# Syclus123/xDeepFM-pytorch

Hardware: AMD Instinct MI355X
Metric: examples/sec (xDeepFM train step, Criteo-shape synthetic, bs=4096 per GPU) (higher is better)
Workload: dtype f32

## Files before the change

### xdeepfm-pytorch_amd/csrc/adam.hip

```cpp
#include "xdfm_internal.h"
#include "finish_batch.h"
#include "adam_math.h"
#include "cin_x3_pack.h"
#include "table_step.h"

#define ADAM_THREADS 256
#define ADAM_BX 512
#define ADAM_BLOCK_ELEMS 8192
#define ADAM_FLUSH_BX 4096



#define ADAM_CHUNK 64
struct AdamDev {
    float* param; float* grad; float* exp_avg; float* exp_avg_sq; const float* step; unsigned char* grad_marks; unsigned char* last;
    long numel; float l2; int flags;
};
static inline AdamDev adam_dev(const xdfm_adam_tensor& t) {
    return AdamDev{t.param, t.grad, t.exp_avg, t.exp_avg_sq, t.step, t.grad_marks, t.last, t.numel, t.l2, t.flags};
}
struct AdamBatch { AdamDev t[ADAM_CHUNK]; int first[ADAM_CHUNK + 1]; };
static_assert(sizeof(AdamBatch) + 128 <= 8192, "the Adam kernels' argument block");

template <bool NT>
// ... 184 lines not shown
__global__ void adam_tick_kernel(int* __restrict__ clock, float* __restrict__ consts, int cap, double lr_arg,
                                 const double* __restrict__ lr_dev, double beta1, double beta2) {
    if (threadIdx.x != 0 || blockIdx.x != 0) return;
    const double lr = lr_dev ? *lr_dev : lr_arg;
    int t = clock[0] + 1;
    if (t >= cap) t = cap - 1;
    clock[0] = t;
    const double step = (double)(clock[1] + t);
    const float ss = (float)(lr / (1.0 - pow(beta1, step)));
    const float bc = (float)sqrt(1.0 - pow(beta2, step));
    const bool ok = bc >= 0.00390625f && bc <= 1.f && ss >= 9.313225746154785e-10f && ss <= 1024.f;
    float* k = consts + ADAM_CONSTS_PER_STEP * t;
    k[0] = ss;
    k[1] = bc;
    k[2] = bc * 4294967296.f;
    k[3] = ok ? adam_exact_rcp(bc) * 2.3283064365386963e-10f : 0.f;
}

__global__ void adam_clock_reset_kernel(int* __restrict__ clock) {
    if (threadIdx.x == 0 && blockIdx.x == 0) { clock[1] += clock[0]; clock[0] = 0; }
}

__device__ __forceinline__ long long adam_backlog_fix(float v) { return (long long)((double)v * ADAM_FIX); }
__device__ __forceinline__ void adam_backlog_add_fix(long long f, unsigned long long* __restrict__ backlog) {
    for (int o = 32; o > 0; o >>= 1) f += __shfl_xor(f, o);
    __shared__ long long part[ADAM_THREADS / 64];
    if ((threadIdx.x & 63) == 0) part[threadIdx.x >> 6] = f;
    __syncthreads();
    if (threadIdx.x == 0) {
        long long tot = 0;
        for (int k = 0; k < ADAM_THREADS / 64; ++k) tot += part[k];
        if (tot) atomicAdd(backlog, (unsigned long long)tot);
    }
}
__device__ __forceinline__ void adam_backlog_add(float v, unsigned long long* __restrict__ backlog) {
    adam_backlog_add_fix(adam_backlog_fix(v), backlog);
}

struct AdamRowsDev {
    float* const* p; float* const* m; float* const* v; unsigned char* const* last; const float* l2;
    float* const* g; unsigned char* const* marks;
};
__device__ __forceinline__ AdamRowsDev adam_rows_pick(bool is_lin, const AdamRowsDev& emb, const AdamRowsDev& lin) {
    AdamRowsDev R;
    R.p = is_lin ? lin.p : emb.p; R.m = is_lin ? lin.m : emb.m; R.v = is_lin ? lin.v : emb.v;
    R.last = is_lin ? lin.last : emb.last; R.l2 = is_lin ? lin.l2 : emb.l2;
    R.g = is_lin ? lin.g : emb.g; R.marks = is_lin ? lin.marks : emb.marks;
    return R;
}

struct AdamClaim { int f; long cc; int old; bool is_lin; };
__device__ __forceinline__ AdamClaim adam_claim_chunk(long idx, const float* __restrict__ X, long ldx, const int* __restrict__ cols,
                                                      const int* __restrict__ vocab, int m, int D, int QE, int QT,
                                                      const AdamRowsDev& emb, const AdamRowsDev& lin, int t, bool need_table) {
    AdamClaim k;
    const int q = (int)(idx % QT);
    const long r = idx / QT;
    k.f = (int)(r % m);
    const long b = r / m;
    const int V = vocab[k.f];
    long id = (long)X[b * ldx + cols[k.f]];
    if (id < 0 || id >= V) id = id < 0 ? 0 : V - 1;
    k.is_lin = q >= QE;
    const AdamRowsDev R = adam_rows_pick(k.is_lin, emb, lin);
    const long w = k.is_lin ? 1 : D;
    const long c0 = id * w / 4, c1 = (id * w + w - 1) / 4;
    k.cc = c0 + (k.is_lin ? 0 : q);
    const long n4 = (long)V * w / 4;
    k.old = -1;
    if (k.cc <= c1 && k.cc < n4 && (!need_table || R.p[k.f] != nullptr))
        k.old = tbl_claim(R.last[k.f], k.cc, t);
    return k;
}

__global__ __launch_bounds__(ADAM_THREADS) void adam_catchup_rows_kernel(
    const float* __restrict__ X, long ldx, int B, const int* __restrict__ cols, const int* __restrict__ vocab, int m, int D,
    AdamRowsDev emb, AdamRowsDev lin, int has_lin, const int* __restrict__ clock, const float* __restrict__ consts,
    double beta1, double beta2, double eps, unsigned long long* __restrict__ backlog, int own_blocks, const X3PackJobs riders) {
    if ((int)blockIdx.x >= own_blocks) { x3_absmax_rider(riders, (long)((int)blockIdx.x - own_blocks)); return; }
    const int t = clock[0];
    const int QE = (D + 3) / 4 + ((D & 3) ? 1 : 0);
    const int QT = QE + (has_lin ? 1 : 0);
    const long idx = (long)blockIdx.x * ADAM_THREADS + threadIdx.x;
    const AdamCoef c = {(float)(1.0 - beta1), (float)beta2, (float)(1.0 - beta2), 0.f, (float)eps};
    const bool eps_ok = c.eps >= ADAM_EPS_MIN && c.eps <= 1.f;
    float zf;
    asm volatile("v_mov_b32 %0, 0" : "=v"(zf));
    AdamClaim k;
    k.old = -1; k.f = 0; k.cc = 0; k.is_lin = false;
    if (t > 0 && idx < (long)B * m * QT) k = adam_claim_chunk(idx, X, ldx, cols, vocab, m, D, QE, QT, emb, lin, t, false);
    const bool act = k.old >= 0;
    const AdamRowsDev R = adam_rows_pick(k.is_lin, emb, lin);
    float4 pa = make_float4(0.f, 0.f, 0.f, 0.f), ma = pa, va = pa;
    float4 *p4 = nullptr, *m4 = nullptr, *v4 = nullptr;
    float l2c = 0.f;
    if (act) {
        p4 = reinterpret_cast<float4*>(R.p[k.f]) + k.cc;
        m4 = reinterpret_cast<float4*>(R.m[k.f]) + k.cc;
        v4 = reinterpret_cast<float4*>(R.v[k.f]) + k.cc;
        pa = *p4; ma = *m4; va = *v4;
        l2c = R.l2[k.f];
    }
    adam_f2 sq2 = {0.f, 0.f};
    adam_replay_span(pa, ma, va, act, k.old, t, consts, 2.f * l2c, zf, c, sq2, eps_ok);
    if (act) { *p4 = pa; *m4 = ma; *v4 = va; }
    adam_backlog_add(l2c * (sq2.x + sq2.y), backlog);
}

__device__ __forceinline__ void adam_apply_rows_body(
    const float* __restrict__ X, long ldx, int B, const int* __restrict__ cols, const int* __restrict__ vocab, int m, int D,
    const AdamRowsDev emb, const AdamRowsDev lin, int has_lin, const int* __restrict__ clock, const float* __restrict__ consts,
    double beta1, double beta2, double eps, unsigned long long* __restrict__ cell, const long bid) {
    const int t = clock[0];
    const int QE = (D + 3) / 4 + ((D & 3) ? 1 : 0);
    const int QT = QE + (has_lin ? 1 : 0);
    const long idx = bid * ADAM_THREADS + threadIdx.x;
    const long nrow = (long)B * m * QT;
    const float ss = consts[ADAM_CONSTS_PER_STEP * t], bc = consts[ADAM_CONSTS_PER_STEP * t + 1];
    const AdamCoef c = {(float)(1.0 - beta1), (float)beta2, (float)(1.0 - beta2), 0.f, (float)eps};
    const bool eps_ok = c.eps >= ADAM_EPS_MIN && c.eps <= 1.f;
    float zf;
    asm volatile("v_mov_b32 %0, 0" : "=v"(zf));
    float sqv = 0.f;
    AdamClaim k;
    k.old = -1; k.f = 0; k.cc = 0; k.is_lin = false;
    if (idx < nrow) k = adam_claim_chunk(idx, X, ldx, cols, vocab, m, D, QE, QT, emb, lin, t, true);
    const bool act = k.old >= 0;
    {
        const AdamRowsDev R = adam_rows_pick(k.is_lin, emb, lin);
        float4 pa = make_float4(0.f, 0.f, 0.f, 0.f), ma = pa, va = pa, ga = pa;
        float4 *p4 = nullptr, *m4 = nullptr, *v4 = nullptr;
        float l2c = 0.f;
        if (act) {
            p4 = reinterpret_cast<float4*>(R.p[k.f]) + k.cc;
            m4 = reinterpret_cast<float4*>(R.m[k.f]) + k.cc;
            v4 = reinterpret_cast<float4*>(R.v[k.f]) + k.cc;
            float4* g4 = reinterpret_cast<float4*>(R.g[k.f]) + k.cc;
            pa = *p4; ma = *m4; va = *v4; ga = *g4;
            *g4 = make_float4(zf, zf, zf, zf);
            R.marks[k.f][k.cc] = 0;
            l2c = R.l2[k.f];
        }
        const float g2 = 2.f * l2c;
        adam_f2 sq2 = {0.f, 0.f};
        adam_replay_span(pa, ma, va, act, k.old, t - 1, consts, g2, zf, c, sq2, eps_ok);
        if (act) {
            float sq = sq2.x + sq2.y;
            adam_four(pa, ma, va, ga, g2, ss, bc, c, sq);
            *p4 = pa; *m4 = ma; *v4 = va;
            sqv = l2c * sq;
        }
    }
    if (idx >= nrow && idx < nrow + 8L * m) {
        const long u = idx - nrow;
        const int kk = (int)(u & 3);
        const int f = (int)((u >> 2) % m);
        const bool is_lin = (u >> 2) >= m;
        if (!is_lin || has_lin) {
            const AdamRowsDev R = adam_rows_pick(is_lin, emb, lin);
            const long numel = (long)vocab[f] * (is_lin ? 1 : D);
            const long e = numel / 4 * 4 + kk;
            if (e < numel && R.p[f] != nullptr) {
                float* p = R.p[f]; float* mm = R.m[f]; float* vv = R.v[f]; float* g = R.g[f];
                const float l2c = R.l2[f];
                float pa = p[e], ma = mm[e], va = vv[e];
                sqv = l2c * (pa * pa);
                adam_one(pa, fmaf(2.f * l2c, pa, g[e]), ma, va, ss, bc, c);
                p[e] = pa; mm[e] = ma; vv[e] = va;
                g[e] = 0.f;
                R.marks[f][e >> 2] = 0;
            }
        }
    }
    adam_backlog_add(sqv, cell);
}
__global__ __launch_bounds__(ADAM_THREADS) void adam_apply_rows_kernel(
    const float* __restrict__ X, long ldx, int B, const int* __restrict__ cols, const int* __restrict__ vocab, int m, int D,
    AdamRowsDev emb, AdamRowsDev lin, int has_lin, const int* __restrict__ clock, const float* __restrict__ consts,
    double beta1, double beta2, double eps, unsigned long long* __restrict__ cell) {
    adam_apply_rows_body(X, ldx, B, cols, vocab, m, D, emb, lin, has_lin, clock, consts, beta1, beta2, eps, cell, (long)blockIdx.x);
}

struct AdamRow { int f; long c0; int nq; bool is_lin; };
__device__ __forceinline__ AdamRow adam_row_of(long idx, bool live, const float* __restrict__ X, long ldx, const int* __restrict__ cols,
                                               const int* __restrict__ vocab, int m, int B, int D, int has_lin) {
    AdamRow r;
    r.f = 0; r.c0 = 0; r.nq = 0; r.is_lin = false;
    const long nE = (long)m * B;
    if (!live || idx >= (has_lin ? 2 * nE : nE)) return r;
    r.is_lin = idx >= nE;
    const long u = r.is_lin ? idx - nE : idx;
    r.f = (int)(u / B);
    const long b = u - (long)r.f * B;
    const int V = vocab[r.f];
    long id = (long)X[b * ldx + cols[r.f]];
    if (id < 0 || id >= V) id = id < 0 ? 0 : V - 1;
    const long w = r.is_lin ? 1 : D;
    r.c0 = id * w / 4;
    const long left = (long)V * w / 4 - r.c0;
    const long want = r.is_lin ? 1 : D / 4;
    r.nq = (int)(left < want ? (left > 0 ? left : 0) : want);
    return r;
}
__device__ __forceinline__ unsigned long long adam_row_claim(const AdamRow& r, unsigned char* last, int q0, int t) {
    const int gn = r.nq - q0 < 8 ? r.nq - q0 : 8;
    if (gn <= 0) return ~0ull;
    if (!r.is_lin) return tbl_claim_row(last, r.c0 + q0, gn, t);
    const int old = tbl_claim(last, r.c0, t);
    return old < 0 ? ~0ull : ((~0ull << 8) | (unsigned long long)old);
}

__global__ __launch_bounds__(ADAM_THREADS) void adam_catchup_by_row_kernel(
    const float* __restrict__ X, long ldx, int B, const int* __restrict__ cols, const int* __restrict__ vocab, int m, int D,
    AdamRowsDev emb, AdamRowsDev lin, int has_lin, const int* __restrict__ clock, const float* __restrict__ consts,
    double beta1, double beta2, double eps, unsigned long long* __restrict__ backlog, int own_blocks, const X3PackJobs riders) {
    if ((int)blockIdx.x >= own_blocks) { x3_absmax_rider(riders, (long)((int)blockIdx.x - own_blocks)); return; }
    const int t = clock[0];
    const int Q = D / 4;
    const long idx = (long)blockIdx.x * ADAM_THREADS + threadIdx.x;
    const AdamCoef c = {(float)(1.0 - beta1), (float)beta2, (float)(1.0 - beta2), 0.f, (float)eps};
    const bool eps_ok = c.eps >= ADAM_EPS_MIN && c.eps <= 1.f;
    float zf;
    asm volatile("v_mov_b32 %0, 0" : "=v"(zf));
    const AdamRow r = adam_row_of(idx, t > 0, X, ldx, cols, vocab, m, B, D, has_lin);
    const AdamRowsDev R = adam_rows_pick(r.is_lin, emb, lin);
    float4 *p4 = nullptr, *m4 = nullptr, *v4 = nullptr;
    unsigned char* last = nullptr;
    float l2c = 0.f;
    if (r.nq > 0) {
        p4 = reinterpret_cast<float4*>(R.p[r.f]) + r.c0;
        m4 = reinterpret_cast<float4*>(R.m[r.f]) + r.c0;
        v4 = reinterpret_cast<float4*>(R.v[r.f]) + r.c0;
        last = R.last[r.f];
        l2c = R.l2[r.f];
    }
    long long fix = 0;
    for (int q0 = 0; q0 < Q; q0 += 8) {
        const unsigned long long olds = adam_row_claim(r, last, q0, t);
        const int turns = Q - q0 < 8 ? Q - q0 : 8;
        for (int j = 0; j < turns; ++j) {
            const int old = (int)((olds >> (8 * j)) & 255ull);
            const bool act = old != 255;
            float4 pa = make_float4(0.f, 0.f, 0.f, 0.f), ma = pa, va = pa;
            if (act) { pa = p4[q0 + j]; ma = m4[q0 + j]; va = v4[q0 + j]; }
            adam_f2 sq2 = {0.f, 0.f};
            adam_replay_span(pa, ma, va, act, old, t, consts, 2.f * l2c, zf, c, sq2, eps_ok);
            if (act) {
                p4[q0 + j] = pa; m4[q0 + j] = ma; v4[q0 + j] = va;
                fix += adam_backlog_fix(l2c * (sq2.x + sq2.y));
            }
        }
    }
    adam_backlog_add_fix(fix, backlog);
}

__device__ __forceinline__ void adam_apply_by_row_body(
    const float* __restrict__ X, long ldx, int B, const int* __restrict__ cols, const int* __restrict__ vocab, int m, int D,
    const AdamRowsDev emb, const AdamRowsDev lin, int has_lin, const int* __restrict__ clock, const float* __restrict__ consts,
    double beta1, double beta2, double eps, unsigned long long* __restrict__ cell, const long bid) {
    const int t = clock[0];
    const int Q = D / 4;
    const long idx = bid * ADAM_THREADS + threadIdx.x;
    const long nrow = (long)B * m * (has_lin ? 2 : 1);
    const float ss = consts[ADAM_CONSTS_PER_STEP * t], bc = consts[ADAM_CONSTS_PER_STEP * t + 1];
    const AdamCoef c = {(float)(1.0 - beta1), (float)beta2, (float)(1.0 - beta2), 0.f, (float)eps};
    const bool eps_ok = c.eps >= ADAM_EPS_MIN && c.eps <= 1.f;
    float zf;
    asm volatile("v_mov_b32 %0, 0" : "=v"(zf));
    long long fix = 0;
    {
        AdamRow r = adam_row_of(idx, true, X, ldx, cols, vocab, m, B, D, has_lin);
        const AdamRowsDev R = adam_rows_pick(r.is_lin, emb, lin);
        float4 *p4 = nullptr, *m4 = nullptr, *v4 = nullptr, *g4 = nullptr;
        unsigned char *last = nullptr, *marks = nullptr;
        float l2c = 0.f;
        if (r.nq > 0 && R.p[r.f] == nullptr) r.nq = 0;
        if (r.nq > 0) {
            p4 = reinterpret_cast<float4*>(R.p[r.f]) + r.c0;
            m4 = reinterpret_cast<float4*>(R.m[r.f]) + r.c0;
            v4 = reinterpret_cast<float4*>(R.v[r.f]) + r.c0;
            g4 = reinterpret_cast<float4*>(R.g[r.f]) + r.c0;
            marks = R.marks[r.f] + r.c0;
            last = R.last[r.f];
            l2c = R.l2[r.f];
        }
        const float g2 = 2.f * l2c;
        for (int q0 = 0; q0 < Q; q0 += 8) {
            const unsigned long long olds = adam_row_claim(r, last, q0, t);
            const int turns = Q - q0 < 8 ? Q - q0 : 8;
            for (int j = 0; j < turns; ++j) {
                const int old = (int)((olds >> (8 * j)) & 255ull);
                const bool act = old != 255;
                float4 pa = make_float4(0.f, 0.f, 0.f, 0.f), ma = pa, va = pa, ga = pa;
                if (act) {
                    pa = p4[q0 + j]; ma = m4[q0 + j]; va = v4[q0 + j]; ga = g4[q0 + j];
                    g4[q0 + j] = make_float4(zf, zf, zf, zf);
                    marks[q0 + j] = 0;
                }
                adam_f2 sq2 = {0.f, 0.f};
                adam_replay_span(pa, ma, va, act, old, t - 1, consts, g2, zf, c, sq2, eps_ok);
                if (act) {
                    float sq = sq2.x + sq2.y;
                    adam_four(pa, ma, va, ga, g2, ss, bc, c, sq);
                    p4[q0 + j] = pa; m4[q0 + j] = ma; v4[q0 + j] = va;
                    fix += adam_backlog_fix(l2c * sq);
                }
            }
        }
    }
    if (idx >= nrow && idx < nrow + 8L * m) {
        const long u = idx - nrow;
        const int kk = (int)(u & 3);
        const int f = (int)((u >> 2) % m);
        const bool is_lin = (u >> 2) >= m;
        if (!is_lin || has_lin) {
            const AdamRowsDev R = adam_rows_pick(is_lin, emb, lin);
            const long numel = (long)vocab[f] * (is_lin ? 1 : D);
            const long e = numel / 4 * 4 + kk;
            if (e < numel && R.p[f] != nullptr) {
                float* p = R.p[f]; float* mm = R.m[f]; float* vv = R.v[f]; float* g = R.g[f];
                const float l2c = R.l2[f];
                float pa = p[e], ma = mm[e], va = vv[e];
                fix += adam_backlog_fix(l2c * (pa * pa));
                adam_one(pa, fmaf(2.f * l2c, pa, g[e]), ma, va, ss, bc, c);
                p[e] = pa; mm[e] = ma; vv[e] = va;
                g[e] = 0.f;
                R.marks[f][e >> 2] = 0;
            }
        }
    }
    adam_backlog_add_fix(fix, cell);
}
__global__ __launch_bounds__(ADAM_THREADS) void adam_apply_by_row_kernel(
    const float* __restrict__ X, long ldx, int B, const int* __restrict__ cols, const int* __restrict__ vocab, int m, int D,
    AdamRowsDev emb, AdamRowsDev lin, int has_lin, const int* __restrict__ clock, const float* __restrict__ consts,
    double beta1, double beta2, double eps, unsigned long long* __restrict__ cell) {
    adam_apply_by_row_body(X, ldx, B, cols, vocab, m, D, emb, lin, has_lin, clock, consts, beta1, beta2, eps, cell, (long)blockIdx.x);
}

struct AdamRowsArgs {
    const float* X; long ldx; int B; const int* cols; const int* vocab; int m; int D;
    AdamRowsDev emb, lin; int has_lin; unsigned long long* cell;
};
static_assert(sizeof(AdamBatch) + sizeof(AdamRowsArgs) + 128 <= 8192, "adam_step_rows_kernel's argument block");
template <bool BY_ROW>
__global__ __launch_bounds__(ADAM_THREADS, 3) void adam_step_rows_kernel(
    const AdamBatch batch, int cnt, int slot0, double lr_arg, const double* __restrict__ lr_dev, double beta1, double beta2, double eps,
    float* __restrict__ l2_part, const int* __restrict__ clock, const float* __restrict__ consts, const AdamRowsArgs r) {
    const int own = batch.first[cnt];
    if ((int)blockIdx.x < own) {
        adam_step_body<true>(batch, cnt, slot0, lr_arg, lr_dev, beta1, beta2, eps, l2_part, clock, consts, (int)blockIdx.x);
        return;
    }
    const long bid = (long)blockIdx.x - own;
    if constexpr (BY_ROW)
        adam_apply_by_row_body(r.X, r.ldx, r.B, r.cols, r.vocab, r.m, r.D, r.emb, r.lin, r.has_lin, clock, consts, beta1, beta2, eps, r.cell, bid);
    else
        adam_apply_rows_body(r.X, r.ldx, r.B, r.cols, r.vocab, r.m, r.D, r.emb, r.lin, r.has_lin, clock, consts, beta1, beta2, eps, r.cell, bid);
}

__global__ void adam_rows_finish_kernel(unsigned long long* __restrict__ cell, float* __restrict__ l2_value) {
    if (threadIdx.x == 0 && blockIdx.x == 0) adam_rows_finish_one(cell, l2_value);
}
int xdfm_adam_rows_finish(unsigned long long* cell, float* l2_value, hipStream_t st) {
    FinishJob j{};
    j.kind = FJ_ADAM_ROWS; j.blocks = 1;
    j.cell = cell; j.out = l2_value;
    bool taken = false;
    if (int rc = xdfm_finish_defer(j, st, &taken)) return rc;
    if (!taken) hipLaunchKernelGGL(adam_rows_finish_kernel, dim3(1), dim3(64), 0, st, cell, l2_value);
    return XDFM_OK;
}

__global__ __launch_bounds__(ADAM_THREADS) void adam_flush_kernel(const AdamBatch batch, int cnt, const int* __restrict__ clock,
                                                                  const float* __restrict__ consts, double beta1, double beta2,
                                                                  double eps, unsigned long long* __restrict__ backlog) {
    int ti = 0;
    for (int k = 1; k < cnt; ++k) ti += (int)blockIdx.x >= batch.first[k] ? 1 : 0;
    const int lb = (int)blockIdx.x - batch.first[ti];
    const int nb = batch.first[ti + 1] - batch.first[ti];
    const AdamDev& d = batch.t[ti];
    const int t = clock[0];
    float4* p4 = reinterpret_cast<float4*>(d.param);
    float4* m4 = reinterpret_cast<float4*>(d.exp_avg);
    float4* v4 = reinterpret_cast<float4*>(d.exp_avg_sq);
    unsigned char* __restrict__ last = d.last;
    const long n4 = d.numel / 4;
    const float l2c = d.l2;
    const float g2 = 2.f * l2c;
    float zf;
    asm volatile("v_mov_b32 %0, 0" : "=v"(zf));
    const AdamCoef c = {(float)(1.0 - beta1), (float)beta2, (float)(1.0 - beta2), 0.f, (float)eps};
    adam_f2 sq2 = {0.f, 0.f};
    const bool eps_ok = c.eps >= ADAM_EPS_MIN && c.eps <= 1.f;
    for (long base = (long)lb * ADAM_THREADS; base < n4; base += (long)nb * ADAM_THREADS) {
        const long i = base + threadIdx.x;
        const bool in = i < n4;
        const int old = in ? (int)last[i] : 0;
        const bool act = in && old < t;
        float4 pa = make_float4(0.f, 0.f, 0.f, 0.f), ma = pa, va = pa;
        if (act) { pa = tbl_ld<true>(p4 + i); ma = tbl_ld<true>(m4 + i); va = tbl_ld<true>(v4 + i); }
        adam_replay_span(pa, ma, va, act, old, t, consts, g2, zf, c, sq2, eps_ok);
        if (act) { tbl_st<true>(p4 + i, pa); tbl_st<true>(m4 + i, ma); tbl_st<true>(v4 + i, va); }
        if (in && old) last[i] = 0;
    }
    adam_backlog_add(l2c * (sq2.x + sq2.y), backlog);
}

__device__ __forceinline__ unsigned long long adam_mix(unsigned long long z) {
    z += 0x9e3779b97f4a7c15ull;
    z = (z ^ (z >> 30)) * 0xbf58476d1ce4e5b9ull;
    z = (z ^ (z >> 27)) * 0x94d049bb133111ebull;
    return z ^ (z >> 31);
}
__device__ __forceinline__ float adam_rand_float(unsigned long long h, int emin, int emax, bool sign) {
    const int e = emin + (int)((h >> 32) % (unsigned)(emax - emin));
    const unsigned bits = ((unsigned)(e + 127) << 23) | ((unsigned)h & 0x7fffffu) | ((sign && ((h >> 60) & 1)) ? 0x80000000u : 0u);
    return __uint_as_float(bits);
}
__device__ __forceinline__ AdamStepConst adam_const_for(double lr, double beta1, double beta2, double step) {
    AdamStepConst k;
    k.ss = (float)(lr / (1.0 - pow(beta1, step)));
    k.bc = (float)sqrt(1.0 - pow(beta2, step));
    k.c2 = k.bc * 4294967296.f;
    k.rc2 = adam_exact_rcp(k.bc) * 2.3283064365386963e-10f;
    return k;
}
__global__ __launch_bounds__(256) void adam_selftest_kernel(int mode, unsigned long long base, unsigned long long n,
                                                            unsigned long long seed, double lr, double beta1, double beta2, double eps,
                                                            unsigned long long* __restrict__ out) {
#pragma clang fp contract(off)
    const unsigned long long idx = base + (unsigned long long)blockIdx.x * 256 + threadIdx.x;
    unsigned long long bad = 0, done = 0, what = 0;
    if (idx < n) {
        if (mode == 0) {
            const float x = __uint_as_float((unsigned)idx);
            if (x > 0.f && x < ADAM_V_MAX) {
                const float x2 = x * 18446744073709551616.f;
                const float fast = adam_sqrt_scaled2(adam_f2{x2, x2}).x, ref = sqrtf(x) * 4294967296.f;
                done = 1; bad = __float_as_uint(fast) != __float_as_uint(ref); what = idx;
            }
        } else if (mode == 1) {
            const unsigned mant = (unsigned)(idx & 0xffffffull);
            const unsigned long long tt = (idx >> 24) + 1;
            const float bc = tt <= 256 ? (float)sqrt(1.0 - pow(beta2, (double)tt)) : adam_rand_float(adam_mix(seed + tt), -8, 0, false);
            const float S = __uint_as_float(0x3f800000u + mant);
            const float s2 = S * 4294967296.f;
            const float fast = adam_div_const2(adam_f2{s2, s2}, bc * 4294967296.f, adam_exact_rcp(bc) * 2.3283064365386963e-10f).y;
            const float ref = S / bc;
            done = 1; bad = __float_as_uint(fast) != __float_as_uint(ref); what = idx;
        } else if (mode == 2) {
            const unsigned long long h0 = adam_mix(seed + 2 * idx), h1 = adam_mix(seed + 2 * idx + 1);
            const float d = adam_rand_float(h0, -40, 40, false);
            float nn = adam_rand_float(h1, -80, 40, true);
            if ((h1 >> 40) % 1021 == 0) nn = 0.f;
            if ((h1 >> 40) % 1021 == 1) nn = __uint_as_float(((h0 >> 61) & 1) ? 0x17800000u : 0x537fffffu);
            const float fast = adam_div2(adam_f2{nn, nn}, adam_f2{d, d}).x, ref = nn / d;
            done = 1; bad = __float_as_uint(fast) != __float_as_uint(ref) && !(fast == 0.f && ref == 0.f);
            what = ((unsigned long long)__float_as_uint(nn) << 32) | __float_as_uint(d);
        } else {
            const AdamCoef c = {(float)(1.0 - beta1), (float)beta2, (float)(1.0 - beta2), 0.f, (float)eps};
            const bool eps_ok = c.eps >= ADAM_EPS_MIN && c.eps <= 1.f;
            float zf;
            asm volatile("v_mov_b32 %0, 0" : "=v"(zf));
            float pv[4], mv[4], vv[4];
            for (int e = 0; e < 4; ++e) {
                const unsigned long long h = adam_mix(seed + 16 * idx + e), h2 = adam_mix(h), h3 = adam_mix(h2);
                pv[e] = adam_rand_float(h, -30, 8, true);
                mv[e] = adam_rand_float(h2, -60, 4, true);
                vv[e] = adam_rand_float(h3, -100, 10, false);
                const unsigned sel = (unsigned)((h >> 48) % 97);
                if (sel == 0) pv[e] = 0.f;
                if (sel == 1) { mv[e] = 0.f; vv[e] = 0.f; }
                if (sel == 2) pv[e] = __uint_as_float(0x00000fffu);
                if (sel == 3) { pv[e] = 3e30f; vv[e] = 1e35f; }
                if (sel == 4) mv[e] = __uint_as_float(0x00400000u);
                if (sel == 5) vv[e] = __uint_as_float(0x00000001u);
            }
            const float g2 = (adam_mix(seed + idx) & 7) == 0 ? 0.f : 2e-5f;
            float4 pf = make_float4(pv[0], pv[1], pv[2], pv[3]), mf = make_float4(mv[0], mv[1], mv[2], mv[3]),
                   vf = make_float4(vv[0], vv[1], vv[2], vv[3]);
            for (int st = 1; st <= 6 && !bad; ++st) {
                const AdamStepConst k = adam_const_for(lr, beta1, beta2, (double)(st + (idx % 50) * 7));
                float4 pr = pf, mr = mf, vr = vf;
                adam_f2 sq2 = {0.f, 0.f};
                adam_replay4(pf, mf, vf, k, g2, zf, c, sq2, eps_ok);
                float* a[3] = {&pr.x, &mr.x, &vr.x};
                for (int e = 0; e < 4; ++e) adam_one(a[0][e], fmaf(g2, a[0][e], zf), a[1][e], a[2][e], k.ss, k.bc, c);
                const float* f[3] = {&pf.x, &mf.x, &vf.x};
                for (int q = 0; q < 3; ++q)
                    for (int e = 0; e < 4; ++e) {
                        const float x = f[q][e], y = a[q][e];
                        if (__float_as_uint(x) != __float_as_uint(y) && !(x != x && y != y) && !(x == 0.f && y == 0.f)) bad = 1;
                    }
                done += 1;
                what = idx * 8 + st;
            }
        }
    }
    if (done) atomicAdd(&out[0], done);
    if (bad) { atomicAdd(&out[1], 1ull); atomicMax(&out[2], what); }
}

static int adam_clock_ok(const char* what, const xdfm_adam_clock* clk) {
    XDFM_REQUIRE(clk && clk->clock && clk->consts && clk->cap > 2 && clk->cap <= 256, "%s: bad clock", what);
    return XDFM_OK;
}

static bool adam_by_row(int D) {
    const bool by_row = D % 4 == 0 && xdfm_opt(OPT_ADAM_ROWS) != 0;
    xdfm_opt_note(OPT_LAST_ADAM_ROWS, by_row ? 1 : 0);
    return by_row;
}

extern "C" {

size_t xdfm_adam_step_ws_elems(int T) { return T > 0 ? (size_t)T * ADAM_BX : 0; }

int xdfm_adam_step(const xdfm_adam_tensor* tensors, int T, double lr, double beta1, double beta2, double eps,
                   float* l2_ws, float* l2_value, void* stream) {
    return xdfm_adam_step_lr(tensors, T, lr, nullptr, beta1, beta2, eps, l2_ws, l2_value, stream);
}

static int adam_step_impl(const xdfm_adam_tensor* tensors, int T, const xdfm_adam_clock* clk, double lr, const double* lr_dev,
                          double beta1, double beta2, double eps, float* l2_ws, float* l2_value, void* stream,
                          const AdamRowsArgs* rows = nullptr, bool rows_by_row = false, int rows_blocks = 0);

int xdfm_adam_step_lr(const xdfm_adam_tensor* tensors, int T, double lr, const double* lr_dev, double beta1, double beta2,
                      double eps, float* l2_ws, float* l2_value, void* stream) {
    return adam_step_impl(tensors, T, nullptr, lr, lr_dev, beta1, beta2, eps, l2_ws, l2_value, stream);
}

int xdfm_adam_step_deferred(const xdfm_adam_tensor* tensors, int T, const xdfm_adam_clock* clk, double lr,
                            const double* lr_dev, double beta1, double beta2, double eps, float* l2_ws, float* l2_value,
                            void* stream) {
    XDFM_REQUIRE(!(clk && clk->clock && clk->consts && clk->cap > 256), "adam_step_deferred: bad clock (cap %d > 256)", clk->cap);
    if (int rc = adam_clock_ok("adam_step_deferred", clk)) return rc;
    return adam_step_impl(tensors, T, clk, lr, lr_dev, beta1, beta2, eps, l2_ws, l2_value, stream);
}

static int adam_step_impl(const xdfm_adam_tensor* tensors, int T, const xdfm_adam_clock* clk, double lr, const double* lr_dev,
                          double beta1, double beta2, double eps, float* l2_ws, float* l2_value, void* stream,
                          const AdamRowsArgs* rows, bool rows_by_row, int rows_blocks) {
    if (int rc = tbl_check_call("adam_step", tensors, T)) return rc;
// ... 164 lines not shown
```

### xdeepfm-pytorch_amd/csrc/adam_math.h

```cpp
#pragma once
#include <hip/hip_runtime.h>

typedef float adam_f2 __attribute__((ext_vector_type(2)));

struct AdamCoef { float w1, b2, w2, lr, eps; };

__device__ __forceinline__ void adam_one(float& p, float g, float& m, float& v, float step_size, float bc2_sqrt, const AdamCoef& c) {
#pragma clang fp contract(off)
    m = fmaf(c.w1, g - m, m);
    v = fmaf(c.w2 * g, g, c.b2 * v);
    const float denom = sqrtf(v) / bc2_sqrt + c.eps;
    p -= step_size * m / denom;
}

__device__ __forceinline__ void adam_four(float4& pa, float4& ma, float4& va, float4 ga, float g2, float step_size, float bc2_sqrt,
                                          const AdamCoef& c, float& sq) {
    sq += (pa.x * pa.x + pa.y * pa.y) + (pa.z * pa.z + pa.w * pa.w);
    ga.x = fmaf(g2, pa.x, ga.x); ga.y = fmaf(g2, pa.y, ga.y); ga.z = fmaf(g2, pa.z, ga.z); ga.w = fmaf(g2, pa.w, ga.w);
    adam_one(pa.x, ga.x, ma.x, va.x, step_size, bc2_sqrt, c); adam_one(pa.y, ga.y, ma.y, va.y, step_size, bc2_sqrt, c);
    adam_one(pa.z, ga.z, ma.z, va.z, step_size, bc2_sqrt, c); adam_one(pa.w, ga.w, ma.w, va.w, step_size, bc2_sqrt, c);
}

struct AdamStepConst { float ss, bc, c2, rc2; };
#define ADAM_CONSTS_PER_STEP 4

__device__ __forceinline__ adam_f2 adam_pkfma(adam_f2 a, adam_f2 b, adam_f2 c) { return __builtin_elementwise_fma(a, b, c); }

__device__ __forceinline__ adam_f2 adam_sqrt_scaled2(adam_f2 x2) {
#pragma clang fp contract(off)
    adam_f2 y;
    y.x = __builtin_amdgcn_rsqf(x2.x);
    y.y = __builtin_amdgcn_rsqf(x2.y);
    const adam_f2 half = {0.5f, 0.5f};
    const adam_f2 s0 = x2 * y, h0 = half * y;
    const adam_f2 r = adam_pkfma(-s0, h0, half);
    const adam_f2 s1 = adam_pkfma(s0, r, s0), h1 = adam_pkfma(h0, r, h0);
    const adam_f2 dd = adam_pkfma(-s1, s1, x2);
    return adam_pkfma(dd, h1, s1);
}

__device__ __forceinline__ adam_f2 adam_div_const2(adam_f2 s, float c2, float rc2) {
#pragma clang fp contract(off)
    const adam_f2 C = {c2, c2}, R = {rc2, rc2};
    const adam_f2 t0 = s * R;
    const adam_f2 r0 = adam_pkfma(-t0, C, s);
    const adam_f2 t1 = adam_pkfma(r0, R, t0);
    const adam_f2 r1 = adam_pkfma(-t1, C, s);
    return adam_pkfma(r1, R, t1);
}

__device__ __forceinline__ adam_f2 adam_div2(adam_f2 n, adam_f2 d) {
#pragma clang fp contract(off)
    adam_f2 y0;
    y0.x = __builtin_amdgcn_rcpf(d.x);
    y0.y = __builtin_amdgcn_rcpf(d.y);
    const adam_f2 one = {1.f, 1.f};
    const adam_f2 e = adam_pkfma(-d, y0, one);
    const adam_f2 y1 = adam_pkfma(e, y0, y0);
    const adam_f2 q0 = n * y1;
    const adam_f2 r0 = adam_pkfma(-d, q0, n);
    const adam_f2 q1 = adam_pkfma(r0, y1, q0);
    const adam_f2 r1 = adam_pkfma(-d, q1, n);
    return adam_pkfma(r1, y1, q1);
}

#define ADAM_V_MAX 4.611686018427388e18f
#define ADAM_M_MIN 8.881784197001252e-16f
#define ADAM_M_MAX 1073741824.0f
#define ADAM_EPS_MIN 9.094947017729282e-13f

__device__ __forceinline__ void adam_replay4(float4& p, float4& m, float4& v, const AdamStepConst& k, float g2, float zf,
                                             const AdamCoef& c, adam_f2& sq2, bool eps_ok) {
#pragma clang fp contract(off)
    adam_f2 pa = {p.x, p.y}, pb = {p.z, p.w};
    sq2 += adam_pkfma(pb, pb, pa * pa);
    const adam_f2 G2 = {g2, g2}, Z = {zf, zf}, W1 = {c.w1, c.w1}, W2 = {c.w2, c.w2}, B2 = {c.b2, c.b2};
    const adam_f2 ga = adam_pkfma(G2, pa, Z), gb = adam_pkfma(G2, pb, Z);
    adam_f2 ma = {m.x, m.y}, mb = {m.z, m.w}, va = {v.x, v.y}, vb = {v.z, v.w};
    const adam_f2 ma1 = adam_pkfma(W1, ga - ma, ma), mb1 = adam_pkfma(W1, gb - mb, mb);
    const adam_f2 va1 = adam_pkfma(W2 * ga, ga, B2 * va), vb1 = adam_pkfma(W2 * gb, gb, B2 * vb);
    const float vmin = fminf(fminf(va1.x, va1.y), fminf(vb1.x, vb1.y)), vmax = fmaxf(fmaxf(va1.x, va1.y), fmaxf(vb1.x, vb1.y));
    const float mmin = fminf(fminf(fabsf(ma1.x), fabsf(ma1.y)), fminf(fabsf(mb1.x), fabsf(mb1.y)));
    const float mmax = fmaxf(fmaxf(fabsf(ma1.x), fabsf(ma1.y)), fmaxf(fabsf(mb1.x), fabsf(mb1.y)));
    const bool fast = vmin > 0.f && vmax < ADAM_V_MAX && mmin >= ADAM_M_MIN && mmax < ADAM_M_MAX;
    if (eps_ok && k.rc2 != 0.f && __builtin_amdgcn_ballot_w64(!fast) == 0) {
        const adam_f2 big = {18446744073709551616.f, 18446744073709551616.f};
        const adam_f2 E = {c.eps, c.eps}, SS = {k.ss, k.ss};
        const adam_f2 sa = adam_sqrt_scaled2(va1 * big), sb = adam_sqrt_scaled2(vb1 * big);
        const adam_f2 da = adam_div_const2(sa, k.c2, k.rc2) + E, db = adam_div_const2(sb, k.c2, k.rc2) + E;
        const adam_f2 neg1 = {-1.f, -1.f};
        pa = adam_pkfma(adam_div2(SS * ma1, da), neg1, pa);
        pb = adam_pkfma(adam_div2(SS * mb1, db), neg1, pb);
        p = make_float4(pa.x, pa.y, pb.x, pb.y);
        m = make_float4(ma1.x, ma1.y, mb1.x, mb1.y);
        v = make_float4(va1.x, va1.y, vb1.x, vb1.y);
    } else {
        adam_one(p.x, ga.x, m.x, v.x, k.ss, k.bc, c); adam_one(p.y, ga.y, m.y, v.y, k.ss, k.bc, c);
        adam_one(p.z, gb.x, m.z, v.z, k.ss, k.bc, c); adam_one(p.w, gb.y, m.w, v.w, k.ss, k.bc, c);
    }
}

__device__ __forceinline__ AdamStepConst adam_step_const(const float* __restrict__ consts, int s) {
    const float4 t = *reinterpret_cast<const float4*>(consts + ADAM_CONSTS_PER_STEP * s);
    return AdamStepConst{t.x, t.y, t.z, t.w};
}

__device__ __forceinline__ void adam_replay_span(float4& p, float4& m, float4& v, bool active, int old, int t_end,
                                                 const float* __restrict__ consts, float g2, float zf, const AdamCoef& c,
                                                 adam_f2& sq2, bool eps_ok) {
    int mn = active ? old : 0x7fffffff;
    for (int o = 32; o > 0; o >>= 1) {
        const int other = __shfl_xor(mn, o);
        mn = other < mn ? other : mn;
    }
    const int first = __builtin_amdgcn_readfirstlane(mn);
    if (first >= t_end) return;
    for (int s = first + 1; s <= t_end; ++s) {
        const AdamStepConst k = adam_step_const(consts, s);
        if (active && s > old) adam_replay4(p, m, v, k, g2, zf, c, sq2, eps_ok);
    }
}

__host__ __device__ inline float adam_exact_rcp(float c) {
    float y = (float)(1.0 / (double)c);
    double best = fabs(1.0 - (double)c * (double)y);
    const float cand[2] = {nextafterf(y, 0.f), nextafterf(y, 3.0e38f)};
    float out = y;
    for (int k = 0; k < 2; ++k) {
        const double r = fabs(1.0 - (double)c * (double)cand[k]);
        if (r < best) { best = r; out = cand[k]; }
    }
    return out;
}
```

Before: 2.184 million.

## Restructure Adam replay math into interleaved packed pairs with uniform coefficients

Reworks the lazy-Adam replay inner step so the sqrt, constant-divide and divide refinements process two packed float pairs side by side, with sched barriers forcing the two chains to interleave. The fast-path range checks become integer bit comparisons combined through wave ballots, and the coefficients are forced into scalar registers with readfirstlane. The full-table flush kernel gains a uniform-loop variant that skips the per-step activity check when all active lanes share the same start step, and it addresses through a shared base plus a lane offset. These changes target ALU latency and VGPR pressure in the catch-up path. The cost is more code and a schedule pinned by barriers, which could stop the compiler from finding a better ordering.

```diff
diff --git a/xdeepfm-pytorch_amd/csrc/adam.hip b/xdeepfm-pytorch_amd/csrc/adam.hip
--- a/xdeepfm-pytorch_amd/csrc/adam.hip
+++ b/xdeepfm-pytorch_amd/csrc/adam.hip
@@ -290,7 +290,7 @@
     const int QE = (D + 3) / 4 + ((D & 3) ? 1 : 0);
     const int QT = QE + (has_lin ? 1 : 0);
     const long idx = (long)blockIdx.x * ADAM_THREADS + threadIdx.x;
-    const AdamCoef c = {(float)(1.0 - beta1), (float)beta2, (float)(1.0 - beta2), 0.f, (float)eps};
+    const AdamCoef c = adam_uniform(AdamCoef{(float)(1.0 - beta1), (float)beta2, (float)(1.0 - beta2), 0.f, (float)eps});
     const bool eps_ok = c.eps >= ADAM_EPS_MIN && c.eps <= 1.f;
     float zf;
     asm volatile("v_mov_b32 %0, 0" : "=v"(zf));
@@ -325,7 +325,7 @@
     const long idx = bid * ADAM_THREADS + threadIdx.x;
     const long nrow = (long)B * m * QT;
     const float ss = consts[ADAM_CONSTS_PER_STEP * t], bc = consts[ADAM_CONSTS_PER_STEP * t + 1];
-    const AdamCoef c = {(float)(1.0 - beta1), (float)beta2, (float)(1.0 - beta2), 0.f, (float)eps};
+    const AdamCoef c = adam_uniform(AdamCoef{(float)(1.0 - beta1), (float)beta2, (float)(1.0 - beta2), 0.f, (float)eps});
     const bool eps_ok = c.eps >= ADAM_EPS_MIN && c.eps <= 1.f;
     float zf;
     asm volatile("v_mov_b32 %0, 0" : "=v"(zf));
@@ -426,7 +426,7 @@
     const int t = clock[0];
     const int Q = D / 4;
     const long idx = (long)blockIdx.x * ADAM_THREADS + threadIdx.x;
-    const AdamCoef c = {(float)(1.0 - beta1), (float)beta2, (float)(1.0 - beta2), 0.f, (float)eps};
+    const AdamCoef c = adam_uniform(AdamCoef{(float)(1.0 - beta1), (float)beta2, (float)(1.0 - beta2), 0.f, (float)eps});
     const bool eps_ok = c.eps >= ADAM_EPS_MIN && c.eps <= 1.f;
     float zf;
     asm volatile("v_mov_b32 %0, 0" : "=v"(zf));
@@ -471,7 +471,7 @@
     const long idx = bid * ADAM_THREADS + threadIdx.x;
     const long nrow = (long)B * m * (has_lin ? 2 : 1);
     const float ss = consts[ADAM_CONSTS_PER_STEP * t], bc = consts[ADAM_CONSTS_PER_STEP * t + 1];
-    const AdamCoef c = {(float)(1.0 - beta1), (float)beta2, (float)(1.0 - beta2), 0.f, (float)eps};
+    const AdamCoef c = adam_uniform(AdamCoef{(float)(1.0 - beta1), (float)beta2, (float)(1.0 - beta2), 0.f, (float)eps});
     const bool eps_ok = c.eps >= ADAM_EPS_MIN && c.eps <= 1.f;
     float zf;
     asm volatile("v_mov_b32 %0, 0" : "=v"(zf));
@@ -595,21 +595,22 @@
     unsigned char* __restrict__ last = d.last;
     const long n4 = d.numel / 4;
     const float l2c = d.l2;
-    const float g2 = 2.f * l2c;
+    const float g2 = adam_uniform(2.f * l2c);
     float zf;
     asm volatile("v_mov_b32 %0, 0" : "=v"(zf));
-    const AdamCoef c = {(float)(1.0 - beta1), (float)beta2, (float)(1.0 - beta2), 0.f, (float)eps};
+    const AdamCoef c = adam_uniform(AdamCoef{(float)(1.0 - beta1), (float)beta2, (float)(1.0 - beta2), 0.f, (float)eps});
     adam_f2 sq2 = {0.f, 0.f};
     const bool eps_ok = c.eps >= ADAM_EPS_MIN && c.eps <= 1.f;
+    const unsigned tx16 = threadIdx.x * 16u;
     for (long base = (long)lb * ADAM_THREADS; base < n4; base += (long)nb * ADAM_THREADS) {
         const long i = base + threadIdx.x;
         const bool in = i < n4;
         const int old = in ? (int)last[i] : 0;
         const bool act = in && old < t;
         float4 pa = make_float4(0.f, 0.f, 0.f, 0.f), ma = pa, va = pa;
-        if (act) { pa = tbl_ld<true>(p4 + i); ma = tbl_ld<true>(m4 + i); va = tbl_ld<true>(v4 + i); }
-        adam_replay_span(pa, ma, va, act, old, t, consts, g2, zf, c, sq2, eps_ok);
-        if (act) { tbl_st<true>(p4 + i, pa); tbl_st<true>(m4 + i, ma); tbl_st<true>(v4 + i, va); }
+        if (act) { pa = tbl_ld<true>(at4(p4 + base, tx16)); ma = tbl_ld<true>(at4(m4 + base, tx16)); va = tbl_ld<true>(at4(v4 + base, tx16)); }
+        adam_replay_span<true>(pa, ma, va, act, old, t, consts, g2, zf, c, sq2, eps_ok);
+        if (act) { tbl_st<true>(at4(p4 + base, tx16), pa); tbl_st<true>(at4(m4 + base, tx16), ma); tbl_st<true>(at4(v4 + base, tx16), va); }
         if (in && old) last[i] = 0;
     }
     adam_backlog_add(l2c * (sq2.x + sq2.y), backlog);
@@ -667,7 +668,7 @@
             done = 1; bad = __float_as_uint(fast) != __float_as_uint(ref) && !(fast == 0.f && ref == 0.f);
             what = ((unsigned long long)__float_as_uint(nn) << 32) | __float_as_uint(d);
         } else {
-            const AdamCoef c = {(float)(1.0 - beta1), (float)beta2, (float)(1.0 - beta2), 0.f, (float)eps};
+            const AdamCoef c = adam_uniform(AdamCoef{(float)(1.0 - beta1), (float)beta2, (float)(1.0 - beta2), 0.f, (float)eps});
             const bool eps_ok = c.eps >= ADAM_EPS_MIN && c.eps <= 1.f;
             float zf;
             asm volatile("v_mov_b32 %0, 0" : "=v"(zf));
diff --git a/xdeepfm-pytorch_amd/csrc/adam_math.h b/xdeepfm-pytorch_amd/csrc/adam_math.h
--- a/xdeepfm-pytorch_amd/csrc/adam_math.h
+++ b/xdeepfm-pytorch_amd/csrc/adam_math.h
@@ -5,12 +5,24 @@
 
 struct AdamCoef { float w1, b2, w2, lr, eps; };
 
-__device__ __forceinline__ void adam_one(float& p, float g, float& m, float& v, float step_size, float bc2_sqrt, const AdamCoef& c) {
+__device__ __forceinline__ float adam_uniform(float x) {
+    asm volatile("" : "+v"(x));
+    return __int_as_float(__builtin_amdgcn_readfirstlane(__float_as_int(x)));
+}
+__device__ __forceinline__ AdamCoef adam_uniform(const AdamCoef& c) {
+    return AdamCoef{adam_uniform(c.w1), adam_uniform(c.b2), adam_uniform(c.w2), adam_uniform(c.lr), adam_uniform(c.eps)};
+}
+
+__device__ __forceinline__ float adam_one_q(float g, float& m, float& v, float step_size, float bc2_sqrt, const AdamCoef& c) {
 #pragma clang fp contract(off)
     m = fmaf(c.w1, g - m, m);
     v = fmaf(c.w2 * g, g, c.b2 * v);
     const float denom = sqrtf(v) / bc2_sqrt + c.eps;
-    p -= step_size * m / denom;
+    return step_size * m / denom;
+}
+__device__ __forceinline__ void adam_one(float& p, float g, float& m, float& v, float step_size, float bc2_sqrt, const AdamCoef& c) {
+#pragma clang fp contract(off)
+    p -= adam_one_q(g, m, v, step_size, bc2_sqrt, c);
 }
 
 __device__ __forceinline__ void adam_four(float4& pa, float4& ma, float4& va, float4 ga, float g2, float step_size, float bc2_sqrt,
@@ -26,78 +38,150 @@
 
 __device__ __forceinline__ adam_f2 adam_pkfma(adam_f2 a, adam_f2 b, adam_f2 c) { return __builtin_elementwise_fma(a, b, c); }
 
+#define ADAM_LOCKSTEP() __builtin_amdgcn_sched_barrier(0)
+
+__device__ __forceinline__ void adam_sqrt_scaled2x2(adam_f2 xa, adam_f2 xb, adam_f2& oa, adam_f2& ob) {
+#pragma clang fp contract(off)
+    adam_f2 ya, yb;
+    ya.x = __builtin_amdgcn_rsqf(xa.x);
+    ya.y = __builtin_amdgcn_rsqf(xa.y);
+    yb.x = __builtin_amdgcn_rsqf(xb.x);
+    yb.y = __builtin_amdgcn_rsqf(xb.y);
+    const adam_f2 half = {0.5f, 0.5f};
+    const adam_f2 s0a = xa * ya, s0b = xb * yb, h0a = half * ya, h0b = half * yb;
+    ADAM_LOCKSTEP();
+    const adam_f2 ra = adam_pkfma(-s0a, h0a, half), rb = adam_pkfma(-s0b, h0b, half);
+    ADAM_LOCKSTEP();
+    const adam_f2 s1a = adam_pkfma(s0a, ra, s0a), s1b = adam_pkfma(s0b, rb, s0b);
+    ADAM_LOCKSTEP();
+    const adam_f2 dda = adam_pkfma(-s1a, s1a, xa), ddb = adam_pkfma(-s1b, s1b, xb);
+    ADAM_LOCKSTEP();
+    oa = adam_pkfma(dda, h0a, s1a);
+    ob = adam_pkfma(ddb, h0b, s1b);
+    ADAM_LOCKSTEP();
+}
 __device__ __forceinline__ adam_f2 adam_sqrt_scaled2(adam_f2 x2) {
-#pragma clang fp contract(off)
-    adam_f2 y;
-    y.x = __builtin_amdgcn_rsqf(x2.x);
-    y.y = __builtin_amdgcn_rsqf(x2.y);
-    const adam_f2 half = {0.5f, 0.5f};
-    const adam_f2 s0 = x2 * y, h0 = half * y;
-    const adam_f2 r = adam_pkfma(-s0, h0, half);
-    const adam_f2 s1 = adam_pkfma(s0, r, s0), h1 = adam_pkfma(h0, r, h0);
-    const adam_f2 dd = adam_pkfma(-s1, s1, x2);
-    return adam_pkfma(dd, h1, s1);
-}
-
+    adam_f2 a, b;
+    adam_sqrt_scaled2x2(x2, x2, a, b);
+    return a;
+}
+
+__device__ __forceinline__ void adam_div_const2x2(adam_f2 sa, adam_f2 sb, float c2, float rc2, adam_f2& oa, adam_f2& ob) {
+#pragma clang fp contract(off)
+    const adam_f2 C = {c2, c2}, R = {rc2, rc2};
+    const adam_f2 t0a = sa * R, t0b = sb * R;
+    ADAM_LOCKSTEP();
+    const adam_f2 r0a = adam_pkfma(-t0a, C, sa), r0b = adam_pkfma(-t0b, C, sb);
+    ADAM_LOCKSTEP();
+    const adam_f2 t1a = adam_pkfma(r0a, R, t0a), t1b = adam_pkfma(r0b, R, t0b);
+    ADAM_LOCKSTEP();
+    const adam_f2 r1a = adam_pkfma(-t1a, C, sa), r1b = adam_pkfma(-t1b, C, sb);
+    ADAM_LOCKSTEP();
+    oa = adam_pkfma(r1a, R, t1a);
+    ob = adam_pkfma(r1b, R, t1b);
+    ADAM_LOCKSTEP();
+}
 __device__ __forceinline__ adam_f2 adam_div_const2(adam_f2 s, float c2, float rc2) {
-#pragma clang fp contract(off)
-    const adam_f2 C = {c2, c2}, R = {rc2, rc2};
-    const adam_f2 t0 = s * R;
-    const adam_f2 r0 = adam_pkfma(-t0, C, s);
-    const adam_f2 t1 = adam_pkfma(r0, R, t0);
-    const adam_f2 r1 = adam_pkfma(-t1, C, s);
-    return adam_pkfma(r1, R, t1);
-}
-
+    adam_f2 a, b;
+    adam_div_const2x2(s, s, c2, rc2, a, b);
+    return b;
+}
+
+__device__ __forceinline__ void adam_div2x2(adam_f2 na, adam_f2 nb, adam_f2 da, adam_f2 db, adam_f2& oa, adam_f2& ob) {
+#pragma clang fp contract(off)
+    adam_f2 y0a, y0b;
+    y0a.x = __builtin_amdgcn_rcpf(da.x);
+    y0a.y = __builtin_amdgcn_rcpf(da.y);
+    y0b.x = __builtin_amdgcn_rcpf(db.x);
+    y0b.y = __builtin_amdgcn_rcpf(db.y);
+    const adam_f2 one = {1.f, 1.f};
+    const adam_f2 ea = adam_pkfma(-da, y0a, one), eb = adam_pkfma(-db, y0b, one);
+    ADAM_LOCKSTEP();
+    const adam_f2 y1a = adam_pkfma(ea, y0a, y0a), y1b = adam_pkfma(eb, y0b, y0b);
+    ADAM_LOCKSTEP();
+    const adam_f2 q0a = na * y1a, q0b = nb * y1b;
+    ADAM_LOCKSTEP();
+    const adam_f2 r0a = adam_pkfma(-da, q0a, na), r0b = adam_pkfma(-db, q0b, nb);
+    ADAM_LOCKSTEP();
+    const adam_f2 q1a = adam_pkfma(r0a, y1a, q0a), q1b = adam_pkfma(r0b, y1b, q0b);
+    ADAM_LOCKSTEP();
+    const adam_f2 r1a = adam_pkfma(-da, q1a, na), r1b = adam_pkfma(-db, q1b, nb);
+    ADAM_LOCKSTEP();
+    oa = adam_pkfma(r1a, y1a, q1a);
+    ob = adam_pkfma(r1b, y1b, q1b);
+    ADAM_LOCKSTEP();
+}
 __device__ __forceinline__ adam_f2 adam_div2(adam_f2 n, adam_f2 d) {
-#pragma clang fp contract(off)
-    adam_f2 y0;
-    y0.x = __builtin_amdgcn_rcpf(d.x);
-    y0.y = __builtin_amdgcn_rcpf(d.y);
-    const adam_f2 one = {1.f, 1.f};
-    const adam_f2 e = adam_pkfma(-d, y0, one);
-    const adam_f2 y1 = adam_pkfma(e, y0, y0);
-    const adam_f2 q0 = n * y1;
-    const adam_f2 r0 = adam_pkfma(-d, q0, n);
-    const adam_f2 q1 = adam_pkfma(r0, y1, q0);
-    const adam_f2 r1 = adam_pkfma(-d, q1, n);
-    return adam_pkfma(r1, y1, q1);
+    adam_f2 a, b;
+    adam_div2x2(n, n, d, d, a, b);
+    return a;
 }
 
 #define ADAM_V_MAX 4.611686018427388e18f
 #define ADAM_M_MIN 8.881784197001252e-16f
 #define ADAM_M_MAX 1073741824.0f
 #define ADAM_EPS_MIN 9.094947017729282e-13f
+#define ADAM_V_MAX_BITS 0x5e800000u
+#define ADAM_MM_MIN_BITS 0x0d800000u
+#define ADAM_MM_MAX_BITS 0x5d800000u
+
+__device__ __forceinline__ unsigned adam_bits_min4(adam_f2 a, adam_f2 b) {
+    const unsigned x = __float_as_uint(a.x), y = __float_as_uint(a.y), z = __float_as_uint(b.x), w = __float_as_uint(b.y);
+    const unsigned t = x < y ? x : y, u = t < z ? t : z;
+    return u < w ? u : w;
+}
+__device__ __forceinline__ unsigned adam_bits_max4(adam_f2 a, adam_f2 b) {
+    const unsigned x = __float_as_uint(a.x), y = __float_as_uint(a.y), z = __float_as_uint(b.x), w = __float_as_uint(b.y);
+    const unsigned t = x > y ? x : y, u = t > z ? t : z;
+    return u > w ? u : w;
+}
+
+__device__ __forceinline__ void adam_replay_pk(adam_f2& pa, adam_f2& pb, adam_f2& ma, adam_f2& mb, adam_f2& va, adam_f2& vb,
+                                               const AdamStepConst& k, float g2, float zf, const AdamCoef& c, adam_f2& sq2,
+                                               bool eps_ok) {
+#pragma clang fp contract(off)
+    sq2 += adam_pkfma(pb, pb, pa * pa);
+    asm volatile("" : "+v"(sq2));
+    const adam_f2 G2 = {g2, g2}, Z = {zf, zf}, W1 = {c.w1, c.w1}, W2 = {c.w2, c.w2}, B2 = {c.b2, c.b2};
+    const adam_f2 ga = adam_pkfma(G2, pa, Z), gb = adam_pkfma(G2, pb, Z);
+    const adam_f2 ma1 = adam_pkfma(W1, ga - ma, ma), mb1 = adam_pkfma(W1, gb - mb, mb);
+    const adam_f2 va1 = adam_pkfma(W2 * ga, ga, B2 * va), vb1 = adam_pkfma(W2 * gb, gb, B2 * vb);
+    bool fast = eps_ok && k.rc2 != 0.f;
+    if (fast) {
+        const adam_f2 qa = ma1 * ma1, qb = mb1 * mb1;
+        const unsigned long long out = __builtin_amdgcn_ballot_w64(adam_bits_min4(va1, vb1) < 1u) |
+                                       __builtin_amdgcn_ballot_w64(adam_bits_max4(va1, vb1) >= ADAM_V_MAX_BITS) |
+                                       __builtin_amdgcn_ballot_w64(adam_bits_min4(qa, qb) < ADAM_MM_MIN_BITS) |
+                                       __builtin_amdgcn_ballot_w64(adam_bits_max4(qa, qb) >= ADAM_MM_MAX_BITS);
+        fast = out == 0;
+    }
+    adam_f2 qa, qb;
+    if (fast) {
+        const adam_f2 big = {18446744073709551616.f, 18446744073709551616.f};
+        const adam_f2 E = {c.eps, c.eps}, SS = {k.ss, k.ss};
+        adam_f2 sa, sb, ta, tb;
+        adam_sqrt_scaled2x2(va1 * big, vb1 * big, sa, sb);
+        adam_div_const2x2(sa, sb, k.c2, k.rc2, ta, tb);
+        adam_div2x2(SS * ma1, SS * mb1, ta + E, tb + E, qa, qb);
+        ma = ma1; mb = mb1; va = va1; vb = vb1;
+    } else {
+        float m0 = ma.x, m1 = ma.y, m2 = mb.x, m3 = mb.y, v0 = va.x, v1 = va.y, v2 = vb.x, v3 = vb.y;
+        const float q0 = adam_one_q(ga.x, m0, v0, k.ss, k.bc, c), q1 = adam_one_q(ga.y, m1, v1, k.ss, k.bc, c);
+        const float q2 = adam_one_q(gb.x, m2, v2, k.ss, k.bc, c), q3 = adam_one_q(gb.y, m3, v3, k.ss, k.bc, c);
+        qa = adam_f2{q0, q1}; qb = adam_f2{q2, q3};
+        ma = adam_f2{m0, m1}; mb = adam_f2{m2, m3}; va = adam_f2{v0, v1}; vb = adam_f2{v2, v3};
+    }
+    pa = pa - qa;
+    pb = pb - qb;
+}
 
 __device__ __forceinline__ void adam_replay4(float4& p, float4& m, float4& v, const AdamStepConst& k, float g2, float zf,
                                              const AdamCoef& c, adam_f2& sq2, bool eps_ok) {
-#pragma clang fp contract(off)
-    adam_f2 pa = {p.x, p.y}, pb = {p.z, p.w};
-    sq2 += adam_pkfma(pb, pb, pa * pa);
-    const adam_f2 G2 = {g2, g2}, Z = {zf, zf}, W1 = {c.w1, c.w1}, W2 = {c.w2, c.w2}, B2 = {c.b2, c.b2};
-    const adam_f2 ga = adam_pkfma(G2, pa, Z), gb = adam_pkfma(G2, pb, Z);
-    adam_f2 ma = {m.x, m.y}, mb = {m.z, m.w}, va = {v.x, v.y}, vb = {v.z, v.w};
-    const adam_f2 ma1 = adam_pkfma(W1, ga - ma, ma), mb1 = adam_pkfma(W1, gb - mb, mb);
-    const adam_f2 va1 = adam_pkfma(W2 * ga, ga, B2 * va), vb1 = adam_pkfma(W2 * gb, gb, B2 * vb);
-    const float vmin = fminf(fminf(va1.x, va1.y), fminf(vb1.x, vb1.y)), vmax = fmaxf(fmaxf(va1.x, va1.y), fmaxf(vb1.x, vb1.y));
-    const float mmin = fminf(fminf(fabsf(ma1.x), fabsf(ma1.y)), fminf(fabsf(mb1.x), fabsf(mb1.y)));
-    const float mmax = fmaxf(fmaxf(fabsf(ma1.x), fabsf(ma1.y)), fmaxf(fabsf(mb1.x), fabsf(mb1.y)));
-    const bool fast = vmin > 0.f && vmax < ADAM_V_MAX && mmin >= ADAM_M_MIN && mmax < ADAM_M_MAX;
-    if (eps_ok && k.rc2 != 0.f && __builtin_amdgcn_ballot_w64(!fast) == 0) {
-        const adam_f2 big = {18446744073709551616.f, 18446744073709551616.f};
-        const adam_f2 E = {c.eps, c.eps}, SS = {k.ss, k.ss};
-        const adam_f2 sa = adam_sqrt_scaled2(va1 * big), sb = adam_sqrt_scaled2(vb1 * big);
-        const adam_f2 da = adam_div_const2(sa, k.c2, k.rc2) + E, db = adam_div_const2(sb, k.c2, k.rc2) + E;
-        const adam_f2 neg1 = {-1.f, -1.f};
-        pa = adam_pkfma(adam_div2(SS * ma1, da), neg1, pa);
-        pb = adam_pkfma(adam_div2(SS * mb1, db), neg1, pb);
-        p = make_float4(pa.x, pa.y, pb.x, pb.y);
-        m = make_float4(ma1.x, ma1.y, mb1.x, mb1.y);
-        v = make_float4(va1.x, va1.y, vb1.x, vb1.y);
-    } else {
-        adam_one(p.x, ga.x, m.x, v.x, k.ss, k.bc, c); adam_one(p.y, ga.y, m.y, v.y, k.ss, k.bc, c);
-        adam_one(p.z, gb.x, m.z, v.z, k.ss, k.bc, c); adam_one(p.w, gb.y, m.w, v.w, k.ss, k.bc, c);
-    }
+    adam_f2 pa = {p.x, p.y}, pb = {p.z, p.w}, ma = {m.x, m.y}, mb = {m.z, m.w}, va = {v.x, v.y}, vb = {v.z, v.w};
+    adam_replay_pk(pa, pb, ma, mb, va, vb, k, g2, zf, c, sq2, eps_ok);
+    p = make_float4(pa.x, pa.y, pb.x, pb.y);
+    m = make_float4(ma.x, ma.y, mb.x, mb.y);
+    v = make_float4(va.x, va.y, vb.x, vb.y);
 }
 
 __device__ __forceinline__ AdamStepConst adam_step_const(const float* __restrict__ consts, int s) {
@@ -105,6 +189,7 @@
     return AdamStepConst{t.x, t.y, t.z, t.w};
 }
 
+template <bool UNIFORM_LOOP = false>
 __device__ __forceinline__ void adam_replay_span(float4& p, float4& m, float4& v, bool active, int old, int t_end,
                                                  const float* __restrict__ consts, float g2, float zf, const AdamCoef& c,
                                                  adam_f2& sq2, bool eps_ok) {
@@ -115,10 +200,20 @@
     }
     const int first = __builtin_amdgcn_readfirstlane(mn);
     if (first >= t_end) return;
-    for (int s = first + 1; s <= t_end; ++s) {
-        const AdamStepConst k = adam_step_const(consts, s);
-        if (active && s > old) adam_replay4(p, m, v, k, g2, zf, c, sq2, eps_ok);
-    }
+    adam_f2 pa = {p.x, p.y}, pb = {p.z, p.w}, ma = {m.x, m.y}, mb = {m.z, m.w}, va = {v.x, v.y}, vb = {v.z, v.w};
+    if (UNIFORM_LOOP && __builtin_amdgcn_ballot_w64(active && old != first) == 0) {
+        if (active)
+            for (int s = first + 1; s <= t_end; ++s)
+                adam_replay_pk(pa, pb, ma, mb, va, vb, adam_step_const(consts, s), g2, zf, c, sq2, eps_ok);
+    } else {
+        for (int s = first + 1; s <= t_end; ++s) {
+            const AdamStepConst k = adam_step_const(consts, s);
+            if (active && s > old) adam_replay_pk(pa, pb, ma, mb, va, vb, k, g2, zf, c, sq2, eps_ok);
+        }
+    }
+    p = make_float4(pa.x, pa.y, pb.x, pb.y);
+    m = make_float4(ma.x, ma.y, mb.x, mb.y);
+    v = make_float4(va.x, va.y, vb.x, vb.y);
 }
 
 __host__ __device__ inline float adam_exact_rcp(float c) {
```

Result: faster. 2.221 million, median of 6 (+1.7%).
